# google-research/rigl

Hardware: NVIDIA H100
Metric: sparse_train_step_images_per_sec_resnet50_erk80 (higher is better)
Workload: dtype bf16

## Files before the change

### include/rigl_b200.h

```cpp
#ifndef RIGL_B200_H_
#define RIGL_B200_H_

#include <stddef.h>
#include <stdint.h>

#if defined(__GNUC__)
#define RIGL_API __attribute__((visibility("default")))
#else
#define RIGL_API
#endif

#ifdef __cplusplus
extern "C" {
#endif

typedef enum {
  RIGL_OK = 0,
  RIGL_ERR_INVALID_ARG = -1,
  RIGL_ERR_CUDA = -2,
  RIGL_ERR_WORKSPACE = -3,
  RIGL_ERR_UNSUPPORTED = -4,
  RIGL_ERR_DRIVER = -5
} rigl_status;

// ... 82 lines not shown

typedef struct {
  float* param;
  float* m;
  float* v;
  const float* grad;
  const uint32_t* mask_bits;
  int64_t n;
  float weight_decay;
  float grad_scale;
} rigl_adam_desc;
typedef struct rigl_adam_plan rigl_adam_plan;
RIGL_API int rigl_adam_plan_create(const rigl_adam_desc* params, int n_params, rigl_adam_plan** out);
RIGL_API int rigl_adam_plan_destroy(rigl_adam_plan* plan);
RIGL_API int rigl_adam_plan_run(rigl_adam_plan* plan, const float* lr_dev, float* powers_dev, float beta1, float beta2,
                                float epsilon, void* stream);

typedef struct {
  int32_t batch, in_h, in_w, cin;
  int32_t out_h, out_w, cout;
  int32_t ksize, stride, pad;
  int32_t x_pitch;
} rigl_conv_desc;

RIGL_API size_t rigl_conv_workspace_bytes(const rigl_conv_desc* d);
RIGL_API int rigl_masked_conv2d_fprop(const rigl_conv_desc* d, const void* x, const void* packed,
                                      void* y_bf16, float* y_f32, const float* bias, void* ws,
                                      size_t ws_bytes, void* stream);
RIGL_API int rigl_bn_partial_rows(void);
RIGL_API int rigl_masked_conv2d_fprop_bnstats(const rigl_conv_desc* d, const void* x, const void* packed,
                                              void* y_bf16, float* bn_partial, int* bn_rows_out, void* ws,
                                              size_t ws_bytes, void* stream);
RIGL_API int rigl_set_bn_stats_always(int on);
RIGL_API int rigl_masked_conv2d_fprop_bnapply(const rigl_conv_desc* d, const void* x, const void* packed,
                                              const void* residual, const float* scale, const float* shift, int relu,
                                              void* y_bf16, void* ws, size_t ws_bytes, void* stream);
RIGL_API int rigl_masked_conv2d_dgrad(const rigl_conv_desc* d, const void* dy, const void* packed,
                                      void* dx, void* ws, size_t ws_bytes, void* stream);
RIGL_API int rigl_conv2d_wgrad_dense(const rigl_conv_desc* d, const void* x, const void* dy,
                                     float* dw, float beta, void* ws, size_t ws_bytes, void* stream);
RIGL_API int rigl_im2col_nhwc(const rigl_conv_desc* d, const void* x, void* out, int64_t out_pitch,
                              void* stream);
RIGL_API int rigl_stem_s2d_supported(const rigl_conv_desc* d);
RIGL_API size_t rigl_stem_s2d_folded_bytes(const rigl_conv_desc* d);
RIGL_API size_t rigl_stem_s2d_packed_bytes(const rigl_conv_desc* d);
RIGL_API size_t rigl_stem_s2d_workspace_bytes(const rigl_conv_desc* d);
RIGL_API int rigl_stem_s2d_fold_input(const rigl_conv_desc* d, const void* x, void* xs, void* stream);
RIGL_API int rigl_stem_s2d_pack_weights(const rigl_conv_desc* d, const float* w_hwio,
                                        const uint32_t* mask_bits, void* packed, void* stream);
RIGL_API int rigl_stem_s2d_fprop(const rigl_conv_desc* d, const void* xs, const void* packed, void* y,
                                 void* stream);
RIGL_API int rigl_stem_s2d_wgrad(const rigl_conv_desc* d, const void* xs, const void* dy, float* dw,
                                 float beta, void* ws, size_t ws_bytes, void* stream);

RIGL_API size_t rigl_bn_workspace_bytes(int64_t rows, int channels);
RIGL_API int rigl_bn_forward_train(const void* y, const void* residual, const float* gamma,
                                   const float* beta, int64_t rows, int channels, float eps,
                                   float momentum, int relu, float* running_mean, float* running_var,
                                   float* save_mean, float* save_rstd, float* save_scale,
                                   float* save_shift, void* out, void* ws, size_t ws_bytes, void* relu_bits,
                                   void* stream);
RIGL_API int rigl_bn_forward_train_partials(const void* y, const void* residual, const float* gamma,
                                            const float* beta, const float* partial, int partial_rows,
                                            int64_t rows, int channels, float eps, float momentum, int relu,
                                            float* running_mean, float* running_var, float* save_mean,
                                            float* save_rstd, float* save_scale, float* save_shift, void* out,
// ... 28 lines not shown
```

### rigl_b200/_cabi.py

```python
import ctypes as C
import os

_HERE = os.path.dirname(os.path.abspath(__file__))
LIB_PATH = os.path.join(_HERE, 'librigl_b200.so')
_lib = None
ABI_VERSION = 202


class RiglError(RuntimeError):
  pass


class LayerDesc(C.Structure):
  _fields_ = [('weights', C.c_void_p), ('score_grow', C.c_void_p), ('mask_bits', C.c_void_p),
              ('noise', C.c_void_p), ('slots', C.c_void_p * 2), ('grow_values', C.c_void_p), ('score_drop', C.c_void_p),
              ('n', C.c_int64), ('n_prune_override', C.c_int32), ('flags', C.c_int32), ('noise_key', C.c_uint32),
              ('reserved', C.c_uint32), ('grad', C.c_void_p)]


class PackDesc(C.Structure):
  _fields_ = [('weights', C.c_void_p), ('mask_bits', C.c_void_p), ('packed', C.c_void_p),
              ('taps', C.c_int32), ('cin', C.c_int32), ('cout', C.c_int32), ('reserved', C.c_int32)]


# ... 19 lines not shown
_vp, _i64, _i32, _f32, _sz = C.c_void_p, C.c_int64, C.c_int, C.c_float, C.c_size_t

SIGNATURES = {
    'rigl_version': (C.c_int, []),
    'rigl_last_error': (C.c_char_p, []),
    'rigl_launch_count': (C.c_uint64, []),
    'rigl_mask_words': (_i64, [_i64]),
    'rigl_mask_pack_f32': (C.c_int, [_vp, _i64, _vp, _vp]),
    'rigl_mask_unpack_f32': (C.c_int, [_vp, _i64, _vp, _vp]),
    'rigl_mask_popcount': (C.c_int, [_vp, _i64, _vp, _vp]),
    'rigl_apply_mask_f32': (C.c_int, [_vp, _vp, _i64, _vp, _f32, _vp]),
    'rigl_mask_plan_create': (C.c_int, [C.POINTER(LayerDesc), _i32, C.POINTER(_vp)]),
    'rigl_mask_plan_destroy': (C.c_int, [_vp]),
    'rigl_mask_plan_workspace_bytes': (_sz, [_vp]),
    'rigl_mask_update_run': (C.c_int, [_vp, _f32, _i32, _f32, _f32, _i32, _vp, _sz, _vp]),
    'rigl_mask_update_run_noise': (C.c_int, [_vp, _f32, _i32, _f32, _f32, _i32, _f32, C.c_uint64, _vp, _sz, _vp]),
    'rigl_mask_noise_fill': (C.c_int, [_vp, _i64, C.c_uint32, _f32, C.c_uint64, _vp]),
    'rigl_mask_plan_read_stats': (C.c_int, [_vp, _vp, C.POINTER(C.c_int32), _vp]),
    'rigl_packed_weights_bytes': (_sz, [_i32, _i32, _i32]),
    'rigl_pack_masked_weights': (C.c_int, [_vp, _vp, _i32, _i32, _i32, _vp, _vp]),
    'rigl_pack_plan_create': (C.c_int, [C.POINTER(PackDesc), _i32, C.POINTER(_vp)]),
    'rigl_pack_plan_destroy': (C.c_int, [_vp]),
    'rigl_pack_plan_run': (C.c_int, [_vp, _vp]),
    'rigl_sgd_plan_create': (C.c_int, [C.POINTER(SgdDesc), _i32, C.POINTER(_vp)]),
    'rigl_sgd_plan_destroy': (C.c_int, [_vp]),
    'rigl_sgd_plan_run': (C.c_int, [_vp, _vp, _f32, _i32, _vp]),
    'rigl_adam_plan_create': (C.c_int, [C.POINTER(AdamDesc), _i32, C.POINTER(_vp)]),
    'rigl_adam_plan_destroy': (C.c_int, [_vp]),
    'rigl_adam_plan_run': (C.c_int, [_vp, _vp, _vp, _f32, _f32, _f32, _vp]),
    'rigl_conv_workspace_bytes': (_sz, [C.POINTER(ConvDesc)]),
    'rigl_masked_conv2d_fprop': (C.c_int, [C.POINTER(ConvDesc), _vp, _vp, _vp, _vp, _vp, _vp, _sz, _vp]),
    'rigl_bn_partial_rows': (C.c_int, []),
    'rigl_set_bn_stats_always': (C.c_int, [_i32]),
    'rigl_masked_conv2d_fprop_bnstats': (C.c_int, [C.POINTER(ConvDesc), _vp, _vp, _vp, _vp, C.POINTER(C.c_int), _vp, _sz, _vp]),
    'rigl_masked_conv2d_fprop_bnapply': (C.c_int, [C.POINTER(ConvDesc), _vp, _vp, _vp, _vp, _vp, _i32, _vp, _vp, _sz,
                                                   _vp]),
    'rigl_masked_conv2d_dgrad': (C.c_int, [C.POINTER(ConvDesc), _vp, _vp, _vp, _vp, _sz, _vp]),
    'rigl_conv2d_wgrad_dense': (C.c_int, [C.POINTER(ConvDesc), _vp, _vp, _vp, _f32, _vp, _sz, _vp]),
    'rigl_im2col_nhwc': (C.c_int, [C.POINTER(ConvDesc), _vp, _vp, _i64, _vp]),
    'rigl_stem_s2d_supported': (C.c_int, [C.POINTER(ConvDesc)]),
    'rigl_stem_s2d_folded_bytes': (_sz, [C.POINTER(ConvDesc)]),
    'rigl_stem_s2d_packed_bytes': (_sz, [C.POINTER(ConvDesc)]),
    'rigl_stem_s2d_workspace_bytes': (_sz, [C.POINTER(ConvDesc)]),
    'rigl_stem_s2d_fold_input': (C.c_int, [C.POINTER(ConvDesc), _vp, _vp, _vp]),
    'rigl_stem_s2d_pack_weights': (C.c_int, [C.POINTER(ConvDesc), _vp, _vp, _vp, _vp]),
    'rigl_stem_s2d_fprop': (C.c_int, [C.POINTER(ConvDesc), _vp, _vp, _vp, _vp]),
    'rigl_stem_s2d_wgrad': (C.c_int, [C.POINTER(ConvDesc), _vp, _vp, _vp, _f32, _vp, _sz, _vp]),
    'rigl_bn_workspace_bytes': (_sz, [_i64, _i32]),
    'rigl_bn_forward_train': (C.c_int, [_vp, _vp, _vp, _vp, _i64, _i32, _f32, _f32, _i32, _vp, _vp, _vp, _vp,
                                        _vp, _vp, _vp, _vp, _sz, _vp, _vp]),
    'rigl_bn_forward_train_partials': (C.c_int, [_vp, _vp, _vp, _vp, _vp, _i32, _i64, _i32, _f32, _f32, _i32, _vp, _vp,
                                                 _vp, _vp, _vp, _vp, _vp, _vp, _vp]),
    'rigl_bn_apply': (C.c_int, [_vp, _vp, _vp, _vp, _i64, _i32, _i32, _vp, _vp]),
    'rigl_bn_backward': (C.c_int, [_vp, _vp, _vp, _vp, _vp, _vp, _vp, _i64, _i32, _i32, _vp, _vp, _vp, _vp,
                                   _vp, _sz, _vp, _vp]),
    'rigl_depthwise3x3_workspace_bytes': (_sz, [_i32, _i32, _i32, _i32, _i32]),
    'rigl_depthwise3x3_fprop': (C.c_int, [_vp, _vp, _i32, _i32, _i32, _i32, _i32, _vp, _vp]),
    'rigl_depthwise3x3_dgrad': (C.c_int, [_vp, _vp, _i32, _i32, _i32, _i32, _i32, _vp, _vp]),
    'rigl_depthwise3x3_wgrad': (C.c_int, [_vp, _vp, _i32, _i32, _i32, _i32, _i32, _vp, _f32, _vp, _sz, _vp]),
    'rigl_maxpool_same_forward': (C.c_int, [_vp, _i32, _i32, _i32, _i32, _i32, _i32, _vp, _vp, _vp]),
    'rigl_maxpool_same_backward': (C.c_int, [_vp, _vp, _i32, _i32, _i32, _i32, _i32, _i32, _vp, _vp]),
    'rigl_set_force_simt': (C.c_int, [_i32]),
}


def lib():
# ... 31 lines not shown
```

### rigl_b200/csrc/conv_api.cu

```cuda
#include <stdlib.h>

#include "common.cuh"
#include "conv_common.cuh"

namespace rigl {

static int g_force_simt = -1;

static bool force_simt() {
  if (g_force_simt < 0) {
    const char* e = getenv("RIGL_FORCE_SIMT");
    g_force_simt = (e && e[0] == '1') ? 1 : 0;
  }
  return g_force_simt == 1;
}

int geom_from_desc(const rigl_conv_desc* d, ConvGeom* g) {
  RIGL_REQUIRE(d != nullptr, "null conv desc");
  RIGL_REQUIRE(d->batch > 0 && d->in_h > 0 && d->in_w > 0 && d->cin > 0 && d->cout > 0 && d->ksize > 0 &&
                   d->stride > 0 && d->pad >= 0,
               "conv desc: non-positive dimension");
  RIGL_REQUIRE(d->pad < d->ksize && d->out_h > 0 && d->out_w > 0 &&
                   (d->out_h - 1) * d->stride - d->pad < d->in_h && (d->out_w - 1) * d->stride - d->pad < d->in_w,
               "conv desc: output %dx%d inconsistent with input %dx%d, k=%d, stride=%d, pad=%d", d->out_h,
// ... 71 lines not shown

extern "C" int rigl_set_force_simt(int on) {
  g_force_simt = on ? 1 : 0;
  return RIGL_OK;
}

extern "C" size_t rigl_conv_workspace_bytes(const rigl_conv_desc* d) {
  ConvGeom g;
  if (geom_from_desc(d, &g) != RIGL_OK) return 0;
  return tc_workspace_bytes(g);
}

extern "C" int rigl_masked_conv2d_fprop(const rigl_conv_desc* d, const void* x, const void* packed,
                                        void* y_bf16, float* y_f32, const float* bias, void* ws,
                                        size_t ws_bytes, void* stream) {
  ConvGeom g;
  int rc = geom_from_desc(d, &g);
  if (rc != RIGL_OK) return rc;
  RIGL_REQUIRE(x && packed && (y_bf16 || y_f32), "rigl_masked_conv2d_fprop: null tensor");
  const PackedLayout L = packed_layout(g.taps(), g.cin, g.cout);
  if (!force_simt() && tc_supported(g, 0))
    return tc_fprop(g, x, packed, y_bf16, y_f32, bias, ws, ws_bytes, (cudaStream_t)stream);
  return simt_fprop(g, x, static_cast<const uint8_t*>(packed) + L.off_dgrad, y_bf16, y_f32, bias,
                    (cudaStream_t)stream);
}

extern "C" int rigl_bn_partial_rows(void) { return tc_max_ctas(); }

extern "C" int rigl_set_bn_stats_always(int on) {
  tc_set_bn_stats_always(on != 0);
  return RIGL_OK;
}

extern "C" int rigl_masked_conv2d_fprop_bnstats(const rigl_conv_desc* d, const void* x, const void* packed,
                                                void* y_bf16, float* bn_partial, int* bn_rows_out, void* ws,
                                                size_t ws_bytes, void* stream) {
  ConvGeom g;
  int rc = geom_from_desc(d, &g);
  if (rc != RIGL_OK) return rc;
  RIGL_REQUIRE(x && packed && y_bf16 && bn_partial && bn_rows_out, "rigl_masked_conv2d_fprop_bnstats: null argument");
  if (force_simt() || !tc_supported(g, 0)) {
    set_error("rigl_masked_conv2d_fprop_bnstats: shape not on the tensor-core path");
    return RIGL_ERR_UNSUPPORTED;
  }
  return tc_fprop(g, x, packed, y_bf16, nullptr, nullptr, ws, ws_bytes, (cudaStream_t)stream, bn_partial, bn_rows_out);
}

extern "C" int rigl_masked_conv2d_fprop_bnapply(const rigl_conv_desc* d, const void* x, const void* packed,
                                                const void* residual, const float* scale, const float* shift, int relu,
                                                void* y_bf16, void* ws, size_t ws_bytes, void* stream) {
  ConvGeom g;
  int rc = geom_from_desc(d, &g);
  if (rc != RIGL_OK) return rc;
  RIGL_REQUIRE(x && packed && scale && shift && y_bf16, "rigl_masked_conv2d_fprop_bnapply: null argument");
  RIGL_REQUIRE(g.cout % 8 == 0, "rigl_masked_conv2d_fprop_bnapply: cout %d is not a multiple of 8", g.cout);
  RIGL_REQUIRE(aligned16(x) && aligned16(y_bf16) && aligned16(residual),
               "rigl_masked_conv2d_fprop_bnapply: tensors must be 16-byte aligned");
  if (force_simt() || !tc_supported(g, 0)) {
    set_error("rigl_masked_conv2d_fprop_bnapply: shape not on the K-major tensor-core kernel");
    return RIGL_ERR_UNSUPPORTED;
  }
  const BnApplyArgs bn = {residual, scale, shift, relu};
  return tc_fprop(g, x, packed, y_bf16, nullptr, nullptr, ws, ws_bytes, (cudaStream_t)stream, nullptr, nullptr, &bn);
}

extern "C" int rigl_masked_conv2d_dgrad(const rigl_conv_desc* d, const void* dy, const void* packed,
// ... 23 lines not shown
```

### rigl_b200/csrc/conv_common.cuh

```cuda
#pragma once
#include <stdint.h>
#include <stddef.h>

#include "../../include/rigl_b200.h"

namespace rigl {

struct ConvGeom {
  int batch, in_h, in_w, cin;
  int out_h, out_w, cout;
  int ksize, stride, pad;
  int cin_pad, cout_pad;
  int x_pitch;
  __host__ __device__ int64_t out_pixels() const { return (int64_t)batch * out_h * out_w; }
  __host__ __device__ int64_t in_pixels() const { return (int64_t)batch * in_h * in_w; }
  __host__ __device__ int taps() const { return ksize * ksize; }
};

inline int round_up8(int v) { return (v + 7) / 8 * 8; }

struct PackedLayout {
  size_t off_fprop, off_dgrad, off_nnz, total;
  int cin_pad, cout_pad, n_tiles, k_tiles;
};
// ... 4 lines not shown
  L.cout_pad = round_up8(cout);
  L.n_tiles = (cout + 63) / 64;
  L.k_tiles = (cin + 63) / 64;
  auto up = [](size_t v) { return (v + 255) / 256 * 256; };
  L.off_fprop = 0;
  L.off_dgrad = up((size_t)taps * cout * L.cin_pad * 2);
  L.off_nnz = L.off_dgrad + up((size_t)taps * cin * L.cout_pad * 2);
  L.total = L.off_nnz + up((size_t)taps * L.n_tiles * L.k_tiles * 4);
  return L;
}

int geom_from_desc(const rigl_conv_desc* d, ConvGeom* g);

int simt_fprop(const ConvGeom& g, const void* x, const void* w_dgrad, void* y, float* y_f32,
               const float* bias, cudaStream_t s);
int simt_dgrad(const ConvGeom& g, const void* dy, const void* w_fprop, void* dx, cudaStream_t s);
int simt_wgrad(const ConvGeom& g, const void* x, const void* dy, float* dw, float beta, cudaStream_t s);
int simt_im2col(const ConvGeom& g, const void* x, void* out, int64_t out_pitch, cudaStream_t s);

struct BnApplyArgs {
  const void* residual;
  const float* scale;
  const float* shift;
  int relu;
};

bool tc_supported(const ConvGeom& g, int which );
size_t tc_workspace_bytes(const ConvGeom& g);
int tc_fprop(const ConvGeom& g, const void* x, const void* packed, void* y, float* y_f32,
             const float* bias, void* ws, size_t ws_bytes, cudaStream_t s, float* bn_partial = nullptr,
             int* bn_rows = nullptr, const BnApplyArgs* bn_apply = nullptr);
int tc_max_ctas();
void tc_set_bn_stats_always(bool on);
int tc_dgrad(const ConvGeom& g, const void* dy, const void* packed, void* dx, void* ws,
             size_t ws_bytes, cudaStream_t s);
int tc_wgrad(const ConvGeom& g, const void* x, const void* dy, float* dw, float beta, void* ws,
             size_t ws_bytes, cudaStream_t s);

bool s2d_supported(const ConvGeom& g);
size_t s2d_folded_bytes(const ConvGeom& g);
size_t s2d_packed_bytes(const ConvGeom& g);
size_t s2d_workspace_bytes(const ConvGeom& g);
int s2d_fold(const ConvGeom& g, const void* x, void* xs, cudaStream_t s);
int s2d_pack(const ConvGeom& g, const float* w, const uint32_t* bits, void* packed, cudaStream_t s);
int s2d_fprop(const ConvGeom& g, const void* xs, const void* packed, void* y, cudaStream_t s);
int s2d_wgrad(const ConvGeom& g, const void* xs, const void* dy, float* dw, float beta, void* ws, size_t ws_bytes,
              cudaStream_t s);

}
```

### rigl_b200/csrc/igemm_tc.cu

```cuda
#include <cuda.h>
#include <cuda_bf16.h>

#include <stdio.h>
#include <stdlib.h>

#include <mutex>

#include "common.cuh"
#include "conv_common.cuh"
#include "tc_ptx.cuh"

namespace rigl {

using namespace ptx;

constexpr int kMaxTaps = 9;
constexpr int kBM = 128;
constexpr int kBK = 64;
constexpr int kThreads = 384;
constexpr int kConsumerWarp0 = 4;
constexpr int kConsumerWarps = 8;
constexpr int kConsumerThreads = 256;

struct TapInfo {
// ... 123 lines not shown
      const uint32_t dst = slab + (uint32_t)r * 128u + (uint32_t)((jj ^ (r & 7)) << 4) + (uint32_t)(lane & 3) * 4u;
      const float2 f = __bfloat1622float2(__floats2bfloat162_rn(d[e], d[e + 1]));
      float a = fmaf(f.x, sc0, sh0), b = fmaf(f.y, sc1, sh1);
      if (ep.residual) {
        uint32_t rw;
        asm volatile("ld.shared.b32 %0, [%1];" : "=r"(rw) : "r"(dst) : "memory");
        a += __uint_as_float(rw << 16);
        b += __uint_as_float(rw & 0xffff0000u);
      }
      if (ep.relu) { a = fmaxf(a, 0.f); b = fmaxf(b, 0.f); }
      __nv_bfloat162 v = __floats2bfloat162_rn(a, b);
      const uint32_t w = (h ? ok1 : ok0) ? *reinterpret_cast<uint32_t*>(&v) : 0u;
      asm volatile("st.shared.b32 [%0], %1;" ::"r"(dst), "r"(w) : "memory");
    }
  }
}

template <int R>
__device__ __forceinline__ void zero_acc(float (&d)[R]) {
#pragma unroll
  for (int i = 0; i < R; ++i) d[i] = 0.f;
}

template <int CL>
__device__ __forceinline__ void release_stage(uint32_t bar) {
  if (CL == 1) {
    mbar_arrive(bar);
  } else {
#pragma unroll
    for (int c = 0; c < CL; ++c) mbar_arrive_cluster(bar, (uint32_t)c);
  }
}

template <int BN, int STAGES, int CL, bool kBnApply>
__device__ __forceinline__ void kmajor_body(const TMaps4& amaps, const CUtensorMap& bmap, const CUtensorMap& omap,
                                            const IgemmParams& p, const CUtensorMap* rmap, const BnEpilogue& ep) {
  extern __shared__ __align__(1024) uint8_t smem_raw[];
  constexpr uint32_t kABytes = kBM * kBK * 2;
  constexpr uint32_t kBBytes = BN * kBK * 2;
  constexpr uint32_t kStageBytes = kABytes + kBBytes;
  constexpr uint32_t kSlabBytes = kBM * 64 * 2;
  const uint32_t smem_base = (smem_u32(smem_raw) + 1023u) & ~1023u;
  const uint32_t out_base = smem_base + STAGES * kStageBytes;
  const uint32_t bar_base = out_base + 2 * kSlabBytes;
  auto full_bar = [&](int s) { return bar_base + 8u * s; };
  auto empty_bar = [&](int s) { return bar_base + 8u * (STAGES + s); };
  const uint32_t res_bar = bar_base + 8u * (2 * STAGES);

  __shared__ uint32_t live_prod[kLiveWords], live_cons[2][2][kLiveWords];
  const int warp = threadIdx.x >> 5, lane = threadIdx.x & 31;
  if (threadIdx.x == 0) {
    for (int i = 0; i < 4; ++i) prefetch_tmap(&amaps.a[i]);
    prefetch_tmap(&bmap);
    if (p.tma_store) prefetch_tmap(&omap);
    for (int s = 0; s < STAGES; ++s) { mbar_init(full_bar(s), 1); mbar_init(empty_bar(s), kConsumerWarps * CL); }
    if constexpr (kBnApply) {
      mbar_init(res_bar, 1);
      if (ep.residual) prefetch_tmap(rmap);
    }
    fence_barrier_init();
  }
  if (CL > 1) cluster_sync_all(); else __syncthreads();

  const uint32_t cta_rank = CL > 1 ? cluster_ctarank() : 0u;
  const int m_tiles = p.tiles_w * p.tiles_h * p.tiles_n;
  const int total = (m_tiles + CL - 1) / CL * p.n_tiles;
  const int cluster_id = blockIdx.x / CL, n_clusters = gridDim.x / CL;
  constexpr int kBN64 = (BN + 63) / 64;
  constexpr uint16_t kMcMask = (uint16_t)((1u << CL) - 1u);

  if (warp == 0) {
    int stage = 0; uint32_t phase = 0;
    for (int tile = cluster_id; tile < total; tile += n_clusters) {
      const int n_tile = tile % p.n_tiles;
      const int m_tile = (tile / p.n_tiles) * CL + (int)cta_rank;
      const int tw = m_tile % p.tiles_w;
      const int th = (m_tile / p.tiles_w) % p.tiles_h;
      const int tn = m_tile / (p.tiles_w * p.tiles_h);
      const bool masked = build_live_mask<kBN64>(p, n_tile, lane, live_prod);
      int j = 0;
      for (int t = 0; t < p.ntaps; ++t) {
        const TapInfo tap = p.taps[t];
        for (int kb = 0; kb < p.kblks; ++kb, ++j) {
          if (masked && !((live_prod[j >> 5] >> (j & 31)) & 1u)) continue;
          if (CL > 1) mbar_wait_cluster(empty_bar(stage), phase ^ 1u);
          else mbar_wait(empty_bar(stage), phase ^ 1u);
          if (elect_one()) {
            const uint32_t a_dst = smem_base + stage * kStageBytes;
            mbar_arrive_expect_tx(full_bar(stage), kStageBytes);
            tma_load_4d(a_dst, &amaps.a[tap.map_id], full_bar(stage), kb * kBK, tw * p.bw + tap.dw,
                        th * p.bh + tap.dh, tn * p.bn);
            if (CL > 1)
              tma_load_3d_mc(a_dst + kABytes + cta_rank * (uint32_t)(BN / CL) * 128u, &bmap, full_bar(stage),
                             kb * kBK, n_tile * BN + (int)cta_rank * (BN / CL), tap.b_tap, kMcMask);
            else
              tma_load_3d(a_dst + kABytes, &bmap, full_bar(stage), kb * kBK, n_tile * BN, tap.b_tap);
          }
          __syncwarp();
          if (++stage == STAGES) { stage = 0; phase ^= 1u; }
        }
      }
    }
  } else if (warp >= kConsumerWarp0) {
    const int cw = warp - kConsumerWarp0;
    const int wg = cw >> 2;
    const int row = 64 * wg + 16 * (cw & 3) + (lane >> 2);
    const bool issuer = (cw == 0 && lane == 0);
    float acc[BN / 2];
    int stage = 0; uint32_t phase = 0;
    uint32_t slab_ctr = 0;
    uint32_t res_phase = 0;
    float* bn_row = (!kBnApply && p.bn_partial) ? p.bn_partial + (size_t)blockIdx.x * 2 * p.N : nullptr;
    if (bn_row) {
      for (int i = cw * 32 + lane; i < 2 * p.N; i += kConsumerThreads) bn_row[i] = 0.f;
      __threadfence_block();
      named_bar_sync(1, kConsumerThreads);
    }
    int tile_ctr = 0;
    for (int tile = cluster_id; tile < total; tile += n_clusters, ++tile_ctr) {
      const int n_tile = tile % p.n_tiles;
      const int m_tile = (tile / p.n_tiles) * CL + (int)cta_rank;
      uint32_t* live = live_cons[wg][tile_ctr & 1];
      if ((cw & 3) == 0) build_live_mask<kBN64>(p, n_tile, lane, live);
      named_bar_sync(3 + wg, 128);
      const bool masked = live_mask_used(p);
      zero_acc(acc);
      int prev = -1;
      const int nkb = p.ntaps * p.kblks;
      for (int j = 0; j < nkb; ++j) {
        if (masked && !((live[j >> 5] >> (j & 31)) & 1u)) continue;
        mbar_wait(full_bar(stage), phase);
        const uint32_t a_src = smem_base + stage * kStageBytes;
        const uint64_t da = make_smem_desc(a_src + (uint32_t)wg * 64u * 128u, 16, 1024);
        const uint64_t db = make_smem_desc(a_src + kABytes, 16, 1024);
        fence_regs(acc);
        wgmma_fence();
#pragma unroll
        for (int k = 0; k < kBK / 16; ++k)
          Wgmma<BN>::template ss<0, 0>(acc, da + 2 * k, db + 2 * k);
        wgmma_commit();
        wgmma_wait<1>();
        if (prev >= 0 && lane == 0) release_stage<CL>(empty_bar(prev));
        prev = stage;
        if (++stage == STAGES) { stage = 0; phase ^= 1u; }
      }
      wgmma_wait<0>();
      fence_regs(acc);
      if (prev >= 0 && lane == 0) release_stage<CL>(empty_bar(prev));

      const int tw = m_tile % p.tiles_w;
      const int th = (m_tile / p.tiles_w) % p.tiles_h;
      const int tn = m_tile / (p.tiles_w * p.tiles_h);
      bool ok[2]; long long o_pix[2];
#pragma unroll
      for (int h = 0; h < 2; ++h) {
        const int r = row + 8 * h;
        const int pw = tw * p.bw + r % p.bw;
        const int ph = th * p.bh + (r / p.bw) % p.bh;
        const int pn = tn * p.bn + r / (p.bw * p.bh);
        ok[h] = pw < p.GW && ph < p.GH && pn < p.NB;
        o_pix[h] = p.o_off + pn * p.o_sn + ph * p.o_sh + pw * p.o_sw;
      }
      if (kBnApply || p.tma_store) {
#pragma unroll
        for (int s = 0; s < kBN64; ++s) {
          const int co0 = n_tile * BN + 64 * s;
          if (co0 >= p.N) break;
          const uint32_t slab = out_base + (uint32_t)(slab_ctr & 1) * kSlabBytes;
          if (issuer) tma_store_wait_read<1>();
          named_bar_sync(1, kConsumerThreads);
          if constexpr (kBnApply) {
            if (ep.residual) {
              if (issuer) {
                mbar_arrive_expect_tx(res_bar, kSlabBytes);
                tma_load_4d(slab, rmap, res_bar, co0, tw * p.bw, th * p.bh, tn * p.bn);
              }
              mbar_wait(res_bar, res_phase);
              res_phase ^= 1u;
            }
            if (s == 0) stage_slab_bn<0>(acc, slab, row, ok[0], ok[1], lane, ep, co0, p.N);
            else stage_slab_bn<(kBN64 > 1 ? 1 : 0)>(acc, slab, row, ok[0], ok[1], lane, ep, co0, p.N);
          } else {
            if (s == 0) stage_slab<0>(acc, slab, row, ok[0], ok[1], lane);
            else stage_slab<(kBN64 > 1 ? 1 : 0)>(acc, slab, row, ok[0], ok[1], lane);
          }
          fence_proxy_async_smem();
          named_bar_sync(1, kConsumerThreads);
          if (issuer) {
            tma_store_4d(&omap, slab, co0, tw * p.bw, th * p.bh, tn * p.bn);
            tma_store_commit();
          }
          if (bn_row && wg == 0) slab_bn_stats(slab, cw, lane, bn_row, co0, p.N);
          ++slab_ctr;
        }
      } else {
#pragma unroll
        for (int jc = 0; jc < BN / 8; ++jc) {
#pragma unroll
          for (int h = 0; h < 2; ++h) {
#pragma unroll
            for (int e = 0; e < 2; ++e) {
              const int co = n_tile * BN + 8 * jc + 2 * (lane & 3) + e;
              if (ok[h] && co < p.N) {
                float a = acc[4 * jc + 2 * h + e];
                if (p.bias) a += __ldg(p.bias + co);
                if (p.out_bf16) p.out_bf16[o_pix[h] + co] = __float2bfloat16(a);
                if (p.out_f32) p.out_f32[o_pix[h] + co] = a;
              }
            }
          }
        }
      }
    }
    if (p.tma_store && issuer) tma_store_wait_all();
  }
  if (CL > 1) cluster_sync_all();
}

template <int BN, int STAGES, int CL>
__global__ void __launch_bounds__(kThreads, 1)
k_igemm_kmajor(const __grid_constant__ TMaps4 amaps, const __grid_constant__ CUtensorMap bmap,
               const __grid_constant__ CUtensorMap omap, const IgemmParams p) {
  kmajor_body<BN, STAGES, CL, false>(amaps, bmap, omap, p, nullptr, BnEpilogue{});
}

template <int BN, int STAGES, int CL>
__global__ void __launch_bounds__(kThreads, 1)
k_igemm_kmajor_bn(const __grid_constant__ TMaps4 amaps, const __grid_constant__ CUtensorMap bmap,
                  const __grid_constant__ CUtensorMap omap, const IgemmParams p,
                  const __grid_constant__ CUtensorMap rmap, const BnEpilogue ep) {
  kmajor_body<BN, STAGES, CL, true>(amaps, bmap, omap, p, &rmap, ep);
}

struct WgradParams {
  int ntaps;
  TapInfo taps[kMaxTaps];
  int GW, GH, NB;
  int bw, bh, bn;
  int tiles_w, tiles_h, tiles_n;
  int pblocks, splits, pblocks_per_split;
  int ci, co;
  int m_tiles, n_tiles;
  float* out;
  long long split_stride;
};

template <int BN, int STAGES, int CL>
__global__ void __launch_bounds__(kThreads, 1)
k_igemm_wgrad(const __grid_constant__ TMaps4 xmaps, const __grid_constant__ CUtensorMap dymap,
              const WgradParams p) {
  extern __shared__ __align__(1024) uint8_t smem_raw[];
  constexpr uint32_t kABytes = kBM * kBK * 2;
  constexpr uint32_t kBBytes = BN * kBK * 2;
  constexpr uint32_t kStageBytes = kABytes + kBBytes;
  constexpr uint32_t kBox = 64 * 64 * 2;
  constexpr int kBBoxes = BN / 64;
  static_assert(CL == 1 || kBBoxes % CL == 0, "multicast splits the dY boxes between the CTAs");
  constexpr uint16_t kMcMask = (uint16_t)((1u << CL) - 1u);

  const uint32_t smem_base = (smem_u32(smem_raw) + 1023u) & ~1023u;
  const uint32_t bar_base = smem_base + STAGES * kStageBytes;
  auto full_bar = [&](int s) { return bar_base + 8u * s; };
  auto empty_bar = [&](int s) { return bar_base + 8u * (STAGES + s); };

// ... 302 lines not shown

static int kmajor_grid(const IgemmParams& p) {
  const int cl = kmajor_use_mc(p) ? 2 : 1;
  const int m_tiles = p.tiles_w * p.tiles_h * p.tiles_n;
  const int pairs = ((m_tiles + cl - 1) / cl) * p.n_tiles;
  int clusters = g_num_sms / cl;
  if (pairs < clusters) clusters = pairs;
  return clusters * cl;
}

template <int CL, typename Kern, typename... Args>
static int launch_clustered(Kern kern, int grid, size_t smem, cudaStream_t s, Args... args) {
  if (CL == 1) {
    kern<<<(unsigned)grid, kThreads, smem, s>>>(args...);
    return RIGL_OK;
  }
  cudaLaunchConfig_t cfg = {};
  cfg.gridDim = dim3((unsigned)grid);
  cfg.blockDim = dim3(kThreads);
  cfg.dynamicSmemBytes = smem;
  cfg.stream = s;
  cudaLaunchAttribute attr[1];
  attr[0].id = cudaLaunchAttributeClusterDimension;
  attr[0].val.clusterDim.x = CL; attr[0].val.clusterDim.y = 1; attr[0].val.clusterDim.z = 1;
  cfg.attrs = attr;
  cfg.numAttrs = 1;
  RIGL_CUDA(cudaLaunchKernelEx(&cfg, kern, args...));
  return RIGL_OK;
}

template <int BN, int STAGES, int CL>
static int launch_kmajor(const TMaps4& amaps, const CUtensorMap& bmap, const CUtensorMap& omap, const IgemmParams& p,
                         cudaStream_t s, const CUtensorMap* rmap, const BnEpilogue* ep) {
  constexpr size_t smem = (size_t)STAGES * (kBM * kBK * 2 + BN * kBK * 2) + 2 * (kBM * 64 * 2) + 1024 + 256;
  static_assert(smem <= 227 * 1024, "K-major kernel exceeds the shared memory of an SM");
  static_assert(8 * (2 * STAGES + 1) <= 256, "K-major kernel barriers exceed their shared memory");
  if (ep != nullptr) {
    static bool configured_bn = false;
    if (!configured_bn) {
      RIGL_CUDA(cudaFuncSetAttribute(k_igemm_kmajor_bn<BN, STAGES, CL>, cudaFuncAttributeMaxDynamicSharedMemorySize,
                                     (int)smem));
      configured_bn = true;
    }
    const int rc = launch_clustered<CL>(k_igemm_kmajor_bn<BN, STAGES, CL>, kmajor_grid(p), smem, s, amaps, bmap, omap,
                                        p, *rmap, *ep);
    if (rc != RIGL_OK) return rc;
    RIGL_LAUNCH_CHECK("k_igemm_kmajor_bn");
    return RIGL_OK;
  }
  static bool configured = false;
  if (!configured) {
    RIGL_CUDA(cudaFuncSetAttribute(k_igemm_kmajor<BN, STAGES, CL>, cudaFuncAttributeMaxDynamicSharedMemorySize, (int)smem));
    configured = true;
  }
  const int rc = launch_clustered<CL>(k_igemm_kmajor<BN, STAGES, CL>, kmajor_grid(p), smem, s, amaps, bmap, omap, p);
  if (rc != RIGL_OK) return rc;
  RIGL_LAUNCH_CHECK("k_igemm_kmajor");
  return RIGL_OK;
}

static int dispatch_kmajor(int n_out, const TMaps4& amaps, const CUtensorMap& bmap, const CUtensorMap& omap,
                           IgemmParams& p, int bn_tile, cudaStream_t s, const CUtensorMap* rmap = nullptr,
                           const BnEpilogue* ep = nullptr) {
  p.n_tiles = (n_out + bn_tile - 1) / bn_tile;
  const bool mc = kmajor_use_mc(p);
  if (bn_tile == 64)
    return mc ? launch_kmajor<64, 7, 2>(amaps, bmap, omap, p, s, rmap, ep)
              : launch_kmajor<64, 7, 1>(amaps, bmap, omap, p, s, rmap, ep);
  return mc ? launch_kmajor<128, 5, 2>(amaps, bmap, omap, p, s, rmap, ep)
            : launch_kmajor<128, 5, 1>(amaps, bmap, omap, p, s, rmap, ep);
}

static int pick_bn(int n_out) {
  return n_out > 64 ? 128 : 64;
}

void tc_set_bn_stats_always(bool on) { g_bn_stats_always = on; }

int tc_fprop(const ConvGeom& g, const void* x, const void* packed, void* y, float* y_f32, const float* bias,
             void* ws, size_t ws_bytes, cudaStream_t s, float* bn_partial, int* bn_rows, const BnApplyArgs* bn_apply) {
  (void)ws; (void)ws_bytes;
  int rc = ensure_driver();
  if (rc != RIGL_OK) return rc;
  const PackedLayout L = packed_layout(g.taps(), g.cin, g.cout);
  const uint8_t* pk = static_cast<const uint8_t*>(packed);
  {
    HaloParams hp = {};
    if (y != nullptr && y_f32 == nullptr && bias == nullptr && halo_fprop_ok(g, &hp)) {
      if (bn_apply != nullptr) {
        set_error("fused BN apply: layer runs on the halo kernels");
        return RIGL_ERR_UNSUPPORTED;
      }
      if (bn_partial != nullptr) {
        set_error("fused BN statistics: layer runs on the halo kernels");
        return RIGL_ERR_UNSUPPORTED;
      }
      return halo_launch_kmajor(hp, x, g.cin, g.x_pitch, pk + L.off_fprop, L.cin_pad, g.cout, y, g.cout, false, s);
    }
  }
  if (bn_partial != nullptr && !g_bn_stats_always) {
    const int K = g.taps() * g.cin;
    if (!(K >= 512 || (K >= 256 && g.cout <= 128))) {
      set_error("fused BN statistics: not profitable for this shape (K = %d, cout = %d)", K, g.cout);
      return RIGL_ERR_UNSUPPORTED;
    }
  }
  IgemmParams p = {};
  set_pixel_tiling(p, g.out_w, g.out_h, g.batch, 128);
  p.kblks = (g.cin + kBK - 1) / kBK;
  p.N = g.cout;
  p.out_bf16 = static_cast<__nv_bfloat16*>(y); p.out_f32 = y_f32; p.bias = bias;
  p.o_off = 0; p.o_sw = g.cout; p.o_sh = (long long)g.out_w * g.cout; p.o_sn = (long long)g.out_h * g.out_w * g.cout;
  p.nnz = reinterpret_cast<const uint32_t*>(pk + L.off_nnz);
  p.nnz_tap_stride = L.n_tiles * L.k_tiles; p.nnz_n_stride = L.k_tiles; p.nnz_k_stride = 1;
  p.bn_partial = bn_partial;
  TMaps4 amaps;
  const uint32_t abox[4] = {(uint32_t)kBK, (uint32_t)p.bw, (uint32_t)p.bh, (uint32_t)p.bn};
  rc = set_conv_taps(p, &amaps, g, x, abox);
  if (rc != RIGL_OK) return rc;
  const int bn_tile = pick_bn(g.cout);
  CUtensorMap bmap;
  const uint64_t bdims[3] = {(uint64_t)L.cin_pad, (uint64_t)g.cout, (uint64_t)g.taps()};
  const uint64_t bstr[2] = {(uint64_t)L.cin_pad * 2, (uint64_t)g.cout * L.cin_pad * 2};
  const uint32_t bbox[3] = {(uint32_t)kBK, (uint32_t)kmajor_b_rows(p, bn_tile), 1};
  rc = make_tmap(&bmap, pk + L.off_fprop, 3, bdims, bstr, bbox);
  if (rc != RIGL_OK) return rc;
  CUtensorMap omap = bmap;
  p.tma_store = (y != nullptr && y_f32 == nullptr && bias == nullptr && g_tma_store) ? 1 : 0;
  if (p.tma_store) {
    rc = make_act_map(&omap, y, g.batch, g.out_h, g.out_w, g.cout, g.cout, 1, 0, 0, abox);
    if (rc != RIGL_OK) return rc;
  }
  if (bn_partial) {
    if (!p.tma_store) {
      set_error("fused BN statistics need the bf16 TMA-store epilogue");
      return RIGL_ERR_UNSUPPORTED;
    }
    p.bn_partial = bn_partial;
    p.n_tiles = (g.cout + bn_tile - 1) / bn_tile;
    if (bn_rows) *bn_rows = kmajor_grid(p);
  }
  if (bn_apply) {
    if (!p.tma_store) {
      set_error("fused BN apply needs the bf16 TMA-store epilogue");
      return RIGL_ERR_UNSUPPORTED;
    }
    CUtensorMap rmap = omap;
    if (bn_apply->residual) {
      rc = make_act_map(&rmap, bn_apply->residual, g.batch, g.out_h, g.out_w, g.cout, g.cout, 1, 0, 0, abox);
      if (rc != RIGL_OK) return rc;
    }
    const BnEpilogue ep = {bn_apply->scale, bn_apply->shift, bn_apply->relu ? 1 : 0, bn_apply->residual ? 1 : 0};
    return dispatch_kmajor(g.cout, amaps, bmap, omap, p, bn_tile, s, &rmap, &ep);
  }
  return dispatch_kmajor(g.cout, amaps, bmap, omap, p, bn_tile, s);
}

int tc_dgrad(const ConvGeom& g, const void* dy, const void* packed, void* dx, void* ws, size_t ws_bytes,
             cudaStream_t s) {
  (void)ws; (void)ws_bytes;
  int rc = ensure_driver();
  if (rc != RIGL_OK) return rc;
  const PackedLayout L = packed_layout(g.taps(), g.cin, g.cout);
  const uint8_t* pk = static_cast<const uint8_t*>(packed);
  const int st = g.stride;
  {
    HaloParams hp = {};
    if (halo_dgrad_ok(g, &hp))
      return halo_launch_kmajor(hp, dy, g.cout, g.cout, pk + L.off_dgrad, L.cout_pad, g.cin, dx, g.x_pitch, true, s);
  }
  bool need_zero = false;
  for (int ph = 0; ph < st && !need_zero; ++ph)
    for (int pw = 0; pw < st; ++pw) {
      int n = 0;
      for (int kh = 0; kh < g.ksize; ++kh)
        for (int kw = 0; kw < g.ksize; ++kw)
          if (posmod(ph + g.pad - kh, st) == 0 && posmod(pw + g.pad - kw, st) == 0) ++n;
      if (n == 0) need_zero = true;
    }
  if (need_zero) RIGL_CUDA(cudaMemsetAsync(dx, 0, (size_t)g.in_pixels() * g.x_pitch * 2, s));
  for (int ph = 0; ph < st; ++ph)
    for (int pw = 0; pw < st; ++pw) {
      IgemmParams p = {};
      const int gh = (g.in_h - ph + st - 1) / st, gw = (g.in_w - pw + st - 1) / st;
      if (gh <= 0 || gw <= 0) continue;
      p.ntaps = 0;
      for (int kh = 0; kh < g.ksize; ++kh)
        for (int kw = 0; kw < g.ksize; ++kw)
          if (posmod(ph + g.pad - kh, st) == 0 && posmod(pw + g.pad - kw, st) == 0) {
            TapInfo& t = p.taps[p.ntaps++];
            t.map_id = 0; t.dh = (int8_t)((ph + g.pad - kh) / st); t.dw = (int8_t)((pw + g.pad - kw) / st);
            t.b_tap = kh * g.ksize + kw;
          }
      if (p.ntaps == 0) continue;
      set_pixel_tiling(p, gw, gh, g.batch, 128);
      p.kblks = (g.cout + kBK - 1) / kBK;
      p.N = g.cin;
      p.out_bf16 = static_cast<__nv_bfloat16*>(dx);
      p.o_off = ((long long)ph * g.in_w + pw) * g.x_pitch;
      p.o_sw = (long long)st * g.x_pitch; p.o_sh = (long long)st * g.in_w * g.x_pitch;
      p.o_sn = (long long)g.in_h * g.in_w * g.x_pitch;
      p.nnz = reinterpret_cast<const uint32_t*>(pk + L.off_nnz);
      p.nnz_tap_stride = L.n_tiles * L.k_tiles; p.nnz_n_stride = 1; p.nnz_k_stride = L.k_tiles;
      TMaps4 amaps;
      const uint32_t abox[4] = {(uint32_t)kBK, (uint32_t)p.bw, (uint32_t)p.bh, (uint32_t)p.bn};
      rc = make_act_map(&amaps.a[0], dy, g.batch, g.out_h, g.out_w, g.cout, g.cout, 1, 0, 0, abox);
      if (rc != RIGL_OK) return rc;
      for (int i = 1; i < 4; ++i) amaps.a[i] = amaps.a[0];
      const int bn_tile = pick_bn(g.cin);
      CUtensorMap bmap;
      const uint64_t bdims[3] = {(uint64_t)L.cout_pad, (uint64_t)g.cin, (uint64_t)g.taps()};
      const uint64_t bstr[2] = {(uint64_t)L.cout_pad * 2, (uint64_t)g.cin * L.cout_pad * 2};
      const uint32_t bbox[3] = {(uint32_t)kBK, (uint32_t)kmajor_b_rows(p, bn_tile), 1};
      rc = make_tmap(&bmap, pk + L.off_dgrad, 3, bdims, bstr, bbox);
      if (rc != RIGL_OK) return rc;
      CUtensorMap omap = bmap;
      p.tma_store = g_tma_store ? 1 : 0;
      if (p.tma_store) {
        rc = make_act_map(&omap, dx, g.batch, g.in_h, g.in_w, g.cin, g.x_pitch, st, ph, pw, abox);
        if (rc != RIGL_OK) return rc;
      }
      rc = dispatch_kmajor(g.cin, amaps, bmap, omap, p, bn_tile, s);
      if (rc != RIGL_OK) return rc;
    }
  return RIGL_OK;
}

template <int BN, int STAGES, int CL>
static int launch_wgrad_cl(const TMaps4& xmaps, const CUtensorMap& dymap, const WgradParams& p, cudaStream_t s) {
  constexpr size_t smem = (size_t)STAGES * (kBM * kBK * 2 + BN * kBK * 2) + 1024 + 256;
  static_assert(smem <= 227 * 1024, "wgrad kernel exceeds the shared memory of an SM");
  static bool configured = false;
  if (!configured) {
    RIGL_CUDA(cudaFuncSetAttribute(k_igemm_wgrad<BN, STAGES, CL>, cudaFuncAttributeMaxDynamicSharedMemorySize, (int)smem));
    configured = true;
  }
  const int groups = ((p.ntaps * p.m_tiles + CL - 1) / CL) * p.n_tiles * p.splits;
  int clusters = g_num_sms / CL;
  if (groups < clusters) clusters = groups;
  const int rc = launch_clustered<CL>(k_igemm_wgrad<BN, STAGES, CL>, clusters * CL, smem, s, xmaps, dymap, p);
  if (rc != RIGL_OK) return rc;
  RIGL_LAUNCH_CHECK("k_igemm_wgrad");
  return RIGL_OK;
}

template <int BN, int STAGES>
static int launch_wgrad(const TMaps4& xmaps, const CUtensorMap& dymap, const WgradParams& p, cudaStream_t s) {
  if constexpr (BN >= 128) {
    if (g_cluster_mc && p.ntaps * p.m_tiles >= 2) return launch_wgrad_cl<BN, STAGES, 2>(xmaps, dymap, p, s);
  }
  return launch_wgrad_cl<BN, STAGES, 1>(xmaps, dymap, p, s);
}

int tc_wgrad(const ConvGeom& g, const void* x, const void* dy, float* dw, float beta, void* ws, size_t ws_bytes,
             cudaStream_t s) {
// ... 59 lines not shown
```

Baseline: 6655.

## Add 256-row K-major implicit-GEMM tile with wave-cost heuristic selection

Adds a 256-row-per-CTA variant of the K-major implicit-GEMM conv kernel. Each consumer warpgroup issues two WGMMAs per k-step against the same B tile, so every B load is reused across twice as many rows. A cost model picks 256 or 128 rows from wave quantization for fprop (when no BN stats or BN apply is requested) and for dgrad, and a new API can force either mode. The trade-off is double the accumulator registers, larger A stages with only 4 pipeline stages, no cluster multicast, and coarser tiles that can leave SMs idle on small layers.

Result: faster. 6758 (median of 6 runs) (+1.5%).

```diff
diff --git a/include/rigl_b200.h b/include/rigl_b200.h
--- a/include/rigl_b200.h
+++ b/include/rigl_b200.h
@@ -138,6 +138,7 @@
                                               void* y_bf16, float* bn_partial, int* bn_rows_out, void* ws,
                                               size_t ws_bytes, void* stream);
 RIGL_API int rigl_set_bn_stats_always(int on);
+RIGL_API int rigl_set_kmajor_m256(int mode);
 RIGL_API int rigl_masked_conv2d_fprop_bnapply(const rigl_conv_desc* d, const void* x, const void* packed,
                                               const void* residual, const float* scale, const float* shift, int relu,
                                               void* y_bf16, void* ws, size_t ws_bytes, void* stream);
diff --git a/rigl_b200/_cabi.py b/rigl_b200/_cabi.py
--- a/rigl_b200/_cabi.py
+++ b/rigl_b200/_cabi.py
@@ -75,6 +75,7 @@
     'rigl_masked_conv2d_fprop': (C.c_int, [C.POINTER(ConvDesc), _vp, _vp, _vp, _vp, _vp, _vp, _sz, _vp]),
     'rigl_bn_partial_rows': (C.c_int, []),
     'rigl_set_bn_stats_always': (C.c_int, [_i32]),
+    'rigl_set_kmajor_m256': (C.c_int, [_i32]),
     'rigl_masked_conv2d_fprop_bnstats': (C.c_int, [C.POINTER(ConvDesc), _vp, _vp, _vp, _vp, C.POINTER(C.c_int), _vp, _sz, _vp]),
     'rigl_masked_conv2d_fprop_bnapply': (C.c_int, [C.POINTER(ConvDesc), _vp, _vp, _vp, _vp, _vp, _i32, _vp, _vp, _sz,
                                                    _vp]),
diff --git a/rigl_b200/csrc/conv_api.cu b/rigl_b200/csrc/conv_api.cu
--- a/rigl_b200/csrc/conv_api.cu
+++ b/rigl_b200/csrc/conv_api.cu
@@ -127,6 +127,12 @@
   return RIGL_OK;
 }
 
+extern "C" int rigl_set_kmajor_m256(int mode) {
+  RIGL_REQUIRE(mode >= -1 && mode <= 1, "rigl_set_kmajor_m256: mode must be -1, 0 or 1");
+  tc_set_kmajor_m256(mode);
+  return RIGL_OK;
+}
+
 extern "C" int rigl_masked_conv2d_fprop_bnstats(const rigl_conv_desc* d, const void* x, const void* packed,
                                                 void* y_bf16, float* bn_partial, int* bn_rows_out, void* ws,
                                                 size_t ws_bytes, void* stream) {
diff --git a/rigl_b200/csrc/conv_common.cuh b/rigl_b200/csrc/conv_common.cuh
--- a/rigl_b200/csrc/conv_common.cuh
+++ b/rigl_b200/csrc/conv_common.cuh
@@ -60,6 +60,7 @@
              int* bn_rows = nullptr, const BnApplyArgs* bn_apply = nullptr);
 int tc_max_ctas();
 void tc_set_bn_stats_always(bool on);
+void tc_set_kmajor_m256(int mode);
 int tc_dgrad(const ConvGeom& g, const void* dy, const void* packed, void* dx, void* ws,
              size_t ws_bytes, cudaStream_t s);
 int tc_wgrad(const ConvGeom& g, const void* x, const void* dy, float* dw, float beta, void* ws,
diff --git a/rigl_b200/csrc/igemm_tc.cu b/rigl_b200/csrc/igemm_tc.cu
--- a/rigl_b200/csrc/igemm_tc.cu
+++ b/rigl_b200/csrc/igemm_tc.cu
@@ -179,17 +179,30 @@
   }
 }
 
-template <int BN, int STAGES, int CL, bool kBnApply>
+template <int BN, int MW>
+__host__ __device__ constexpr int kmajor_slabs() {
+  return (MW == 2 && BN == 128) ? 1 : 2;
+}
+template <int BN, int STAGES, int MW>
+constexpr size_t kmajor_smem() {
+  return (size_t)STAGES * (MW * kBM * kBK * 2 + BN * kBK * 2) + kmajor_slabs<BN, MW>() * (MW * kBM * 64 * 2) + 1024 +
+         256;
+}
+
+template <int BN, int STAGES, int CL, bool kBnApply, int MW>
 __device__ __forceinline__ void kmajor_body(const TMaps4& amaps, const CUtensorMap& bmap, const CUtensorMap& omap,
                                             const IgemmParams& p, const CUtensorMap* rmap, const BnEpilogue& ep) {
+  static_assert(MW == 1 || (CL == 1 && !kBnApply), "the 256-row tile is single-CTA without the BN-apply epilogue");
   extern __shared__ __align__(1024) uint8_t smem_raw[];
-  constexpr uint32_t kABytes = kBM * kBK * 2;
+  constexpr int kRows = MW * kBM;
+  constexpr uint32_t kABytes = kRows * kBK * 2;
   constexpr uint32_t kBBytes = BN * kBK * 2;
   constexpr uint32_t kStageBytes = kABytes + kBBytes;
-  constexpr uint32_t kSlabBytes = kBM * 64 * 2;
+  constexpr uint32_t kSlabBytes = kRows * 64 * 2;
+  constexpr int kSlabs = kmajor_slabs<BN, MW>();
   const uint32_t smem_base = (smem_u32(smem_raw) + 1023u) & ~1023u;
   const uint32_t out_base = smem_base + STAGES * kStageBytes;
-  const uint32_t bar_base = out_base + 2 * kSlabBytes;
+  const uint32_t bar_base = out_base + kSlabs * kSlabBytes;
   auto full_bar = [&](int s) { return bar_base + 8u * s; };
   auto empty_bar = [&](int s) { return bar_base + 8u * (STAGES + s); };
   const uint32_t res_bar = bar_base + 8u * (2 * STAGES);
@@ -251,9 +264,9 @@
   } else if (warp >= kConsumerWarp0) {
     const int cw = warp - kConsumerWarp0;
     const int wg = cw >> 2;
-    const int row = 64 * wg + 16 * (cw & 3) + (lane >> 2);
+    const int row0 = 64 * MW * wg + 16 * (cw & 3) + (lane >> 2);
     const bool issuer = (cw == 0 && lane == 0);
-    float acc[BN / 2];
+    float acc[MW][BN / 2];
     int stage = 0; uint32_t phase = 0;
     uint32_t slab_ctr = 0;
     uint32_t res_phase = 0;
@@ -271,20 +284,24 @@
       if ((cw & 3) == 0) build_live_mask<kBN64>(p, n_tile, lane, live);
       named_bar_sync(3 + wg, 128);
       const bool masked = live_mask_used(p);
-      zero_acc(acc);
+#pragma unroll
+      for (int m = 0; m < MW; ++m) zero_acc(acc[m]);
       int prev = -1;
       const int nkb = p.ntaps * p.kblks;
       for (int j = 0; j < nkb; ++j) {
         if (masked && !((live[j >> 5] >> (j & 31)) & 1u)) continue;
         mbar_wait(full_bar(stage), phase);
         const uint32_t a_src = smem_base + stage * kStageBytes;
-        const uint64_t da = make_smem_desc(a_src + (uint32_t)wg * 64u * 128u, 16, 1024);
+        const uint64_t da = make_smem_desc(a_src + (uint32_t)(MW * wg) * 64u * 128u, 16, 1024);
         const uint64_t db = make_smem_desc(a_src + kABytes, 16, 1024);
-        fence_regs(acc);
+#pragma unroll
+        for (int m = 0; m < MW; ++m) fence_regs(acc[m]);
         wgmma_fence();
 #pragma unroll
         for (int k = 0; k < kBK / 16; ++k)
-          Wgmma<BN>::template ss<0, 0>(acc, da + 2 * k, db + 2 * k);
+#pragma unroll
+          for (int m = 0; m < MW; ++m)
+            Wgmma<BN>::template ss<0, 0>(acc[m], da + 512 * m + 2 * k, db + 2 * k);
         wgmma_commit();
         wgmma_wait<1>();
         if (prev >= 0 && lane == 0) release_stage<CL>(empty_bar(prev));
@@ -292,29 +309,32 @@
         if (++stage == STAGES) { stage = 0; phase ^= 1u; }
       }
       wgmma_wait<0>();
-      fence_regs(acc);
+#pragma unroll
+      for (int m = 0; m < MW; ++m) fence_regs(acc[m]);
       if (prev >= 0 && lane == 0) release_stage<CL>(empty_bar(prev));
 
       const int tw = m_tile % p.tiles_w;
       const int th = (m_tile / p.tiles_w) % p.tiles_h;
       const int tn = m_tile / (p.tiles_w * p.tiles_h);
-      bool ok[2]; long long o_pix[2];
-#pragma unroll
-      for (int h = 0; h < 2; ++h) {
-        const int r = row + 8 * h;
-        const int pw = tw * p.bw + r % p.bw;
-        const int ph = th * p.bh + (r / p.bw) % p.bh;
-        const int pn = tn * p.bn + r / (p.bw * p.bh);
-        ok[h] = pw < p.GW && ph < p.GH && pn < p.NB;
-        o_pix[h] = p.o_off + pn * p.o_sn + ph * p.o_sh + pw * p.o_sw;
-      }
+      bool ok[MW][2]; long long o_pix[MW][2];
+#pragma unroll
+      for (int m = 0; m < MW; ++m)
+#pragma unroll
+        for (int h = 0; h < 2; ++h) {
+          const int r = row0 + 64 * m + 8 * h;
+          const int pw = tw * p.bw + r % p.bw;
+          const int ph = th * p.bh + (r / p.bw) % p.bh;
+          const int pn = tn * p.bn + r / (p.bw * p.bh);
+          ok[m][h] = pw < p.GW && ph < p.GH && pn < p.NB;
+          o_pix[m][h] = p.o_off + pn * p.o_sn + ph * p.o_sh + pw * p.o_sw;
+        }
       if (kBnApply || p.tma_store) {
 #pragma unroll
         for (int s = 0; s < kBN64; ++s) {
           const int co0 = n_tile * BN + 64 * s;
           if (co0 >= p.N) break;
-          const uint32_t slab = out_base + (uint32_t)(slab_ctr & 1) * kSlabBytes;
-          if (issuer) tma_store_wait_read<1>();
+          const uint32_t slab = out_base + (uint32_t)(slab_ctr % kSlabs) * kSlabBytes;
+          if (issuer) tma_store_wait_read<kSlabs - 1>();
           named_bar_sync(1, kConsumerThreads);
           if constexpr (kBnApply) {
             if (ep.residual) {
@@ -325,11 +345,14 @@
               mbar_wait(res_bar, res_phase);
               res_phase ^= 1u;
             }
-            if (s == 0) stage_slab_bn<0>(acc, slab, row, ok[0], ok[1], lane, ep, co0, p.N);
-            else stage_slab_bn<(kBN64 > 1 ? 1 : 0)>(acc, slab, row, ok[0], ok[1], lane, ep, co0, p.N);
+            if (s == 0) stage_slab_bn<0>(acc[0], slab, row0, ok[0][0], ok[0][1], lane, ep, co0, p.N);
+            else stage_slab_bn<(kBN64 > 1 ? 1 : 0)>(acc[0], slab, row0, ok[0][0], ok[0][1], lane, ep, co0, p.N);
           } else {
-            if (s == 0) stage_slab<0>(acc, slab, row, ok[0], ok[1], lane);
-            else stage_slab<(kBN64 > 1 ? 1 : 0)>(acc, slab, row, ok[0], ok[1], lane);
+#pragma unroll
+            for (int m = 0; m < MW; ++m) {
+              if (s == 0) stage_slab<0>(acc[m], slab, row0 + 64 * m, ok[m][0], ok[m][1], lane);
+              else stage_slab<(kBN64 > 1 ? 1 : 0)>(acc[m], slab, row0 + 64 * m, ok[m][0], ok[m][1], lane);
+            }
           }
           fence_proxy_async_smem();
           named_bar_sync(1, kConsumerThreads);
@@ -337,26 +360,30 @@
             tma_store_4d(&omap, slab, co0, tw * p.bw, th * p.bh, tn * p.bn);
             tma_store_commit();
           }
-          if (bn_row && wg == 0) slab_bn_stats(slab, cw, lane, bn_row, co0, p.N);
+          if (bn_row && wg == 0)
+#pragma unroll
+            for (int hr = 0; hr < MW; ++hr) slab_bn_stats(slab + (uint32_t)hr * kBM * 128u, cw, lane, bn_row, co0, p.N);
           ++slab_ctr;
         }
       } else {
 #pragma unroll
-        for (int jc = 0; jc < BN / 8; ++jc) {
-#pragma unroll
-          for (int h = 0; h < 2; ++h) {
-#pragma unroll
-            for (int e = 0; e < 2; ++e) {
-              const int co = n_tile * BN + 8 * jc + 2 * (lane & 3) + e;
-              if (ok[h] && co < p.N) {
-                float a = acc[4 * jc + 2 * h + e];
-                if (p.bias) a += __ldg(p.bias + co);
-                if (p.out_bf16) p.out_bf16[o_pix[h] + co] = __float2bfloat16(a);
-                if (p.out_f32) p.out_f32[o_pix[h] + co] = a;
+        for (int m = 0; m < MW; ++m)
+#pragma unroll
+          for (int jc = 0; jc < BN / 8; ++jc) {
+#pragma unroll
+            for (int h = 0; h < 2; ++h) {
+#pragma unroll
+              for (int e = 0; e < 2; ++e) {
+                const int co = n_tile * BN + 8 * jc + 2 * (lane & 3) + e;
+                if (ok[m][h] && co < p.N) {
+                  float a = acc[m][4 * jc + 2 * h + e];
+                  if (p.bias) a += __ldg(p.bias + co);
+                  if (p.out_bf16) p.out_bf16[o_pix[m][h] + co] = __float2bfloat16(a);
+                  if (p.out_f32) p.out_f32[o_pix[m][h] + co] = a;
+                }
               }
             }
           }
-        }
       }
     }
     if (p.tma_store && issuer) tma_store_wait_all();
@@ -368,7 +395,14 @@
 __global__ void __launch_bounds__(kThreads, 1)
 k_igemm_kmajor(const __grid_constant__ TMaps4 amaps, const __grid_constant__ CUtensorMap bmap,
                const __grid_constant__ CUtensorMap omap, const IgemmParams p) {
-  kmajor_body<BN, STAGES, CL, false>(amaps, bmap, omap, p, nullptr, BnEpilogue{});
+  kmajor_body<BN, STAGES, CL, false, 1>(amaps, bmap, omap, p, nullptr, BnEpilogue{});
+}
+
+template <int BN, int STAGES>
+__global__ void __launch_bounds__(kThreads, 1)
+k_igemm_kmajor_m256(const __grid_constant__ TMaps4 amaps, const __grid_constant__ CUtensorMap bmap,
+                    const __grid_constant__ CUtensorMap omap, const IgemmParams p) {
+  kmajor_body<BN, STAGES, 1, false, 2>(amaps, bmap, omap, p, nullptr, BnEpilogue{});
 }
 
 template <int BN, int STAGES, int CL>
@@ -376,7 +410,7 @@
 k_igemm_kmajor_bn(const __grid_constant__ TMaps4 amaps, const __grid_constant__ CUtensorMap bmap,
                   const __grid_constant__ CUtensorMap omap, const IgemmParams p,
                   const __grid_constant__ CUtensorMap rmap, const BnEpilogue ep) {
-  kmajor_body<BN, STAGES, CL, true>(amaps, bmap, omap, p, &rmap, ep);
+  kmajor_body<BN, STAGES, CL, true, 1>(amaps, bmap, omap, p, &rmap, ep);
 }
 
 struct WgradParams {
@@ -745,7 +779,7 @@
 template <int BN, int STAGES, int CL>
 static int launch_kmajor(const TMaps4& amaps, const CUtensorMap& bmap, const CUtensorMap& omap, const IgemmParams& p,
                          cudaStream_t s, const CUtensorMap* rmap, const BnEpilogue* ep) {
-  constexpr size_t smem = (size_t)STAGES * (kBM * kBK * 2 + BN * kBK * 2) + 2 * (kBM * 64 * 2) + 1024 + 256;
+  constexpr size_t smem = kmajor_smem<BN, STAGES, 1>();
   static_assert(smem <= 227 * 1024, "K-major kernel exceeds the shared memory of an SM");
   static_assert(8 * (2 * STAGES + 1) <= 256, "K-major kernel barriers exceed their shared memory");
   if (ep != nullptr) {
@@ -772,10 +806,29 @@
   return RIGL_OK;
 }
 
-static int dispatch_kmajor(int n_out, const TMaps4& amaps, const CUtensorMap& bmap, const CUtensorMap& omap,
+template <int BN, int STAGES>
+static int launch_kmajor_m256(const TMaps4& amaps, const CUtensorMap& bmap, const CUtensorMap& omap,
+                              const IgemmParams& p, cudaStream_t s) {
+  constexpr size_t smem = kmajor_smem<BN, STAGES, 2>();
+  static_assert(smem <= 227 * 1024, "K-major kernel exceeds the shared memory of an SM");
+  static bool configured = false;
+  if (!configured) {
+    RIGL_CUDA(cudaFuncSetAttribute(k_igemm_kmajor_m256<BN, STAGES>, cudaFuncAttributeMaxDynamicSharedMemorySize,
+                                   (int)smem));
+    configured = true;
+  }
+  k_igemm_kmajor_m256<BN, STAGES><<<(unsigned)kmajor_grid(p), kThreads, smem, s>>>(amaps, bmap, omap, p);
+  RIGL_LAUNCH_CHECK("k_igemm_kmajor_m256");
+  return RIGL_OK;
+}
+
+static int dispatch_kmajor(int n_out, int rows, const TMaps4& amaps, const CUtensorMap& bmap, const CUtensorMap& omap,
                            IgemmParams& p, int bn_tile, cudaStream_t s, const CUtensorMap* rmap = nullptr,
                            const BnEpilogue* ep = nullptr) {
   p.n_tiles = (n_out + bn_tile - 1) / bn_tile;
+  if (rows == 2 * kBM)
+    return bn_tile == 64 ? launch_kmajor_m256<64, 4>(amaps, bmap, omap, p, s)
+                         : launch_kmajor_m256<128, 4>(amaps, bmap, omap, p, s);
   const bool mc = kmajor_use_mc(p);
   if (bn_tile == 64)
     return mc ? launch_kmajor<64, 7, 2>(amaps, bmap, omap, p, s, rmap, ep)
@@ -788,6 +841,24 @@
   return n_out > 64 ? 128 : 64;
 }
 
+static int g_kmajor_m256 = -1;
+
+static int kmajor_rows(int gw, int gh, int nb, int n_out, bool bn_stats, bool bn_apply) {
+  if (g_cluster_mc || bn_apply) return kBM;
+  if (g_kmajor_m256 >= 0) return g_kmajor_m256 ? 2 * kBM : kBM;
+  if (bn_stats) return kBM;
+  const int bn_tile = pick_bn(n_out);
+  const long long n_tiles = (n_out + bn_tile - 1) / bn_tile;
+  auto cost = [&](int rows) {
+    int bw, bh, bn;
+    choose_box(gw, gh, nb, rows, &bw, &bh, &bn);
+    const long long tiles = (long long)((gw + bw - 1) / bw) * ((gh + bh - 1) / bh) * ((nb + bn - 1) / bn) * n_tiles;
+    return (tiles + g_num_sms - 1) / g_num_sms * rows;
+  };
+  return cost(2 * kBM) <= cost(kBM) ? 2 * kBM : kBM;
+}
+
+void tc_set_kmajor_m256(int mode) { g_kmajor_m256 = mode; }
 void tc_set_bn_stats_always(bool on) { g_bn_stats_always = on; }
 
 int tc_fprop(const ConvGeom& g, const void* x, const void* packed, void* y, float* y_f32, const float* bias,
@@ -819,7 +890,8 @@
     }
   }
   IgemmParams p = {};
-  set_pixel_tiling(p, g.out_w, g.out_h, g.batch, 128);
+  const int rows = kmajor_rows(g.out_w, g.out_h, g.batch, g.cout, bn_partial != nullptr, bn_apply != nullptr);
+  set_pixel_tiling(p, g.out_w, g.out_h, g.batch, rows);
   p.kblks = (g.cin + kBK - 1) / kBK;
   p.N = g.cout;
   p.out_bf16 = static_cast<__nv_bfloat16*>(y); p.out_f32 = y_f32; p.bias = bias;
@@ -864,9 +936,9 @@
       if (rc != RIGL_OK) return rc;
     }
     const BnEpilogue ep = {bn_apply->scale, bn_apply->shift, bn_apply->relu ? 1 : 0, bn_apply->residual ? 1 : 0};
-    return dispatch_kmajor(g.cout, amaps, bmap, omap, p, bn_tile, s, &rmap, &ep);
-  }
-  return dispatch_kmajor(g.cout, amaps, bmap, omap, p, bn_tile, s);
+    return dispatch_kmajor(g.cout, rows, amaps, bmap, omap, p, bn_tile, s, &rmap, &ep);
+  }
+  return dispatch_kmajor(g.cout, rows, amaps, bmap, omap, p, bn_tile, s);
 }
 
 int tc_dgrad(const ConvGeom& g, const void* dy, const void* packed, void* dx, void* ws, size_t ws_bytes,
@@ -906,7 +978,8 @@
             t.b_tap = kh * g.ksize + kw;
           }
       if (p.ntaps == 0) continue;
-      set_pixel_tiling(p, gw, gh, g.batch, 128);
+      const int rows = kmajor_rows(gw, gh, g.batch, g.cin, false, false);
+      set_pixel_tiling(p, gw, gh, g.batch, rows);
       p.kblks = (g.cout + kBK - 1) / kBK;
       p.N = g.cin;
       p.out_bf16 = static_cast<__nv_bfloat16*>(dx);
@@ -933,7 +1006,7 @@
         rc = make_act_map(&omap, dx, g.batch, g.in_h, g.in_w, g.cin, g.x_pitch, st, ph, pw, abox);
         if (rc != RIGL_OK) return rc;
       }
-      rc = dispatch_kmajor(g.cin, amaps, bmap, omap, p, bn_tile, s);
+      rc = dispatch_kmajor(g.cin, rows, amaps, bmap, omap, p, bn_tile, s);
       if (rc != RIGL_OK) return rc;
     }
   return RIGL_OK;
```
